# cvlab-dresden/DSAC

Measured on AMD Instinct MI355X. Metric: hypotheses scored/sec over 640x480 coord map, higher is better.
Workload: dtype f32

## Files before the change

### dsac_amd/csrc/api.hip

```cpp
#include "../../include/dsac_hip.h"
#include "kernels.h"
#include "refstream.h"

#include <hip/hip_runtime.h>
#include <cstdarg>
#include <cstdio>
#include <algorithm>
#include <cstring>
#include <cmath>
#include <deque>
#include <string>
#include <type_traits>
#include <vector>
#if defined(_GLIBCXX_RELEASE) && _GLIBCXX_RELEASE < 11
#define DSAC_RS_DEFAULT_MODE 1
#else
#define DSAC_RS_DEFAULT_MODE 0
#endif

namespace {

thread_local std::string g_last_error;

struct DevBuf {
// ... 43 lines not shown
    dk::FrameDev F{};
    DevBuf frame_xyz, frame_uv;
    std::vector<float> cams_h;
    DevBuf cams_d;
    DevBuf cam_xyz, cam_meta, rgbd_rec, rgbd_soft_part, rgbd_scratch;
    bool have_cam = false;
    GuideTable guide, rgbd_guide;
    DevBuf guide_scratch, rgbd_guide_wm;

    DevBuf rs_states, rs_scratch, rs_small, k6_scratch;
    int rs_threads = 0, rs_mode = DSAC_RS_DEFAULT_MODE;
    int pi_refstream = 0, pi_refstream_discard0 = 0, pi_refstream_attempts = 0;
    int k6_walk_exact = 0;
    int k6_waves = 0;
    int refine_soft_form = -1;
    DevBuf soft_scratch;
    DevBuf staged, staged_lo, staged_split, soft_part, bwd_staged, dRdH, grad_part, g12_part, g6;
    int g6_n = 0;
    std::deque<DevBuf> slots;
    size_t slot_next = 0;
    struct Pending { void* host; const void* dev; size_t bytes; };
    std::vector<Pending> pending;
    dk::K2Opts k2;
    int k2_last[2] = {0, 0};
    dk::K1Opts k1;
    int k1_cus = 0;
    bool device_args = false;
    int seed_stride = 1;
    int k4_variant = -1;
    hipEvent_t k2_wait = nullptr, k2_record = nullptr;

    hipStream_t aux = nullptr, aux2 = nullptr;
    DevBuf slot_staged[2], slot_soft_part[2];
    hipEvent_t slot_ready[2] = {nullptr, nullptr}, slot_free[2] = {nullptr, nullptr}, slot_reduced[2] = {nullptr, nullptr},
               slot_done[2] = {nullptr, nullptr};
    bool slot_free_recorded[2] = {false, false}, slot_reduced_recorded[2] = {false, false}, slot_done_recorded[2] = {false, false};
    bool slot_pending[2] = {false, false};
    int slot_N[2] = {0, 0};
    dk::FrameDev slot_F[2]{};
    hipEvent_t frame_ready = nullptr;

    int pi_defer_tail = 0;
    hipStream_t tail[2] = {nullptr, nullptr};
    hipEvent_t tail_go = nullptr, tail_done[2] = {nullptr, nullptr};
    bool tail_pending[2] = {false, false};
    DevBuf pi_soft[2], pi_scores[2];
// ... 159 lines not shown
    if (sums && !part) return fail(c, DSAC_ERR_INVALID, "k2_stage: the plan writes partial sums and no buffer was given");
    if (gated && c->k2_wait) HIP_TRY(c, hipStreamWaitEvent(st, c->k2_wait, 0));
    dk::K2Call call;
    if (plan.need_split) {
        HIP_TRY(c, c->staged_split.reserve(dk::pose_split_bytes(N)));
        HIP_TRY(c, dk::pose_prep_split(st, N, poses, F, c->staged_split.as<char>(), Nf));
        call.split = c->staged_split.as<char>();
    }
    if (plan.need_lo) {
        HIP_TRY(c, c->staged_lo.reserve((size_t)N * dk::POSE_STRIDE * sizeof(float)));
        HIP_TRY(c, dk::pose_prep_lo(st, N, poses, F, c->staged_lo.as<float>(), Nf));
        call.staged_lo = c->staged_lo.as<float>();
    }
    ProfScope ps(c, 0, true);
    call.poses64 = poses;
    call.diag = c->k2.diag;
    if (ps.on) { call.ev_start = ps.p.a; call.ev_stop = ps.p.b; }
    else call.ev_stop = fallback_stop;
    if (done) *done = call.ev_stop;
    HIP_TRY(c, dk::reproject(st, plan, N, staged, F, clampv, static_cast<float*>(err), tau, beta, sums ? part : nullptr, call));
    ps.commit();
    c->k2_last[0] = plan.form;
    c->k2_last[1] = plan.why;
    if (gated && c->k2_record) HIP_TRY(c, hipEventRecord(c->k2_record, st));
    return DSAC_OK;
}

struct FdStage {
    int skip = 0;
    float eps_hyp = 0.f, eps_obj = 0.f;
    dk::FdLists L{};
    dk::FdReplicas rep{};
};
int fd_stage_check(dsac_ctx* c, const char* who, float sub_sample, const float* eps_hyp, float eps_obj, FdStage* s) {
    if (eps_hyp) {
        if (!(sub_sample > 0.f) || !(*eps_hyp > 0.f) || !(eps_obj > 0.f)) return fail(c, DSAC_ERR_INVALID, "%s: sub_sample, eps_hyp, eps_obj must be > 0", who);
        s->eps_hyp = *eps_hyp;
    } else if (!(sub_sample > 0.f) || !(eps_obj > 0.f)) return fail(c, DSAC_ERR_INVALID, "%s: sub_sample and eps_obj must be > 0", who);
    s->eps_obj = eps_obj;
    s->skip = (int)(1 / sub_sample);
    if (s->skip < 1) return fail(c, DSAC_ERR_INVALID, "%s: sub_sample > 1", who);
    return DSAC_OK;
}
int fd_stage_begin(dsac_ctx* c, FdStage* s, const dk::FdLists& L, const double* init_poses, const int32_t* sets, const int32_t* maps, const int32_t* perm, int steps,
                   int max_inl, int min_inl, float thr, int32_t* obj_pixels, int32_t* n_obj, hipEvent_t planned = nullptr) {
    s->L = L;
// ... 211 lines not shown
        return fail(nullptr, DSAC_ERR_NO_DEVICE, "dsac_create: no HIP device (%s); this engine has no CPU fallback",
                    e != hipSuccess ? hipGetErrorString(e) : "device count 0");
    }
    if (device < 0 || device >= count) return fail(nullptr, DSAC_ERR_INVALID, "dsac_create: device %d out of range [0,%d)", device, count);
    HIP_TRY(nullptr, hipSetDevice(device));
    dsac_ctx* c = new (std::nothrow) dsac_ctx();
    if (!c) return fail(nullptr, DSAC_ERR_ALLOC, "dsac_create: out of host memory");
    c->device = device;
    e = hipGetDeviceProperties(&c->prop, device);
    if (e != hipSuccess) { delete c; return fail(nullptr, DSAC_ERR_HIP, "hipGetDeviceProperties: %s", hipGetErrorString(e)); }
    if (strncmp(c->prop.gcnArchName, "gfx950", 6) != 0) {
        std::string n = c->prop.gcnArchName;
        delete c;
        return fail(nullptr, DSAC_ERR_NO_DEVICE, "dsac_create: device %d is %s; this library carries gfx950 code only", device, n.c_str());
    }
    e = hipStreamCreateWithFlags(&c->stream, hipStreamNonBlocking);
    if (e != hipSuccess) { delete c; return fail(nullptr, DSAC_ERR_HIP, "hipStreamCreate: %s", hipGetErrorString(e)); }
    c->own_stream = true;
    if (const char* v = getenv("DSAC_K2_VARIANT")) c->k2.variant = atoi(v);
    if (const char* v = getenv("DSAC_TAIL_PRIO")) c->tail_prio = atoi(v) != 0;
    if (const char* v = getenv("DSAC_K2_ORDER")) c->k2.pixel_minor = atoi(v) != 0;
    if (const char* v = getenv("DSAC_K2_FLAGS")) c->k2.flags = atoi(v);
    if (const char* v = getenv("DSAC_K2_EXACT_AUTO")) c->k2.exact_auto = atoi(v) != 0;
    if (const char* v = getenv("DSAC_K1_WPB")) c->k1.wpb = atoi(v);
    if (const char* v = getenv("DSAC_K1_PRIO")) c->k1.prio = atoi(v);
    if (const char* v = getenv("DSAC_K1_HPW")) c->k1.hpw = atoi(v);
    if (const char* v = getenv("DSAC_K1_HORN")) c->k1.horn = atoi(v) != 0;
    if (const char* v = getenv("DSAC_K1_MINW")) c->k1.minw = atoi(v);
    if (const char* v = getenv("DSAC_K1_RL")) c->k1.rl = atoi(v) == 1 ? 1 : 4;
    if (const char* v = getenv("DSAC_K1_WIDE")) c->k1.wide = atoi(v);
    if (const char* v = getenv("DSAC_K1_SHARE")) { const int sv = atoi(v); c->k1.share = sv < 0 ? -sv : sv; c->k1.share_always = sv < 0; }
    if (const char* v = getenv("DSAC_K4_VARIANT")) c->k4_variant = atoi(v);
    if (const char* v = getenv("DSAC_K1_CUS")) c->k1_cus = atoi(v);
    *out = c;
    return DSAC_OK;
}

void dsac_destroy(dsac_ctx* c) {
    if (!c) return;
    (void)hipSetDevice(c->device);
    if (c->stream) (void)hipStreamSynchronize(c->stream);
    for (int k = 0; k < 2; k++)
        if (c->tail[k]) (void)hipStreamSynchronize(c->tail[k]);
    if (c->aux) (void)hipStreamSynchronize(c->aux);
    if (c->aux2) (void)hipStreamSynchronize(c->aux2);
    c->frame_xyz.release(); c->frame_uv.release(); c->cams_d.release();
// ... 739 lines not shown
    const int32_t* d_sets;
    double* d_J;
    ARG_TRY(in_arg(c, sets, (size_t)N * 4, &d_sets));
    ARG_TRY(out_arg(c, J, (size_t)N * 72, &d_J));
    HIP_TRY(c, dk::dpnp(c->stream, N, d_sets, c->F, eps, d_J, c->F.frames > 1 ? N / c->F.frames : 0));
    return end_call(c);
}

int dsac_set_option(dsac_ctx* c, const char* key, int value) {
    if (!c || !key) return fail(c, DSAC_ERR_INVALID, "dsac_set_option: NULL argument");
    const std::string k = key;
    if (k == "k2_variant") {
        if (!dk::k2_variant_known(value)) return fail(c, DSAC_ERR_INVALID, "dsac_set_option: unknown K2 kernel form %d", value);
        c->k2.variant = value;
    }
    else if (k == "k2_order") c->k2.pixel_minor = value != 0;
    else if (k == "k2_flags") c->k2.flags = value;
    else if (k == "k2_diag") c->k2.diag = value;
    else if (k == "k2_exact_auto") c->k2.exact_auto = value != 0;
    else if (k == "k2_f16_store") {
        if (value != 0 && value != 1) return fail(c, DSAC_ERR_INVALID, "dsac_set_option: k2_f16_store (both 16-bit builds, binary16 and bfloat16) is 0 (8-byte stores) or 1 (16-byte stores after a lane exchange)");
        c->k2.f16_store = value;
    }
    else if (k == "k6_walk_exact") c->k6_walk_exact = value != 0;
    else if (k == "k6_scan_tune") {
        const int g = value & 255, chunk = (value >> 8) & 0xffff;
        if ((g != 0 && g != 1 && g != 2 && g != 4) || chunk % 256 != 0 || (value >> 25) != 0) return fail(c, DSAC_ERR_INVALID, "dsac_set_option: k6_scan_tune is g | chunk << 8 | noskip << 24 with g in {0, 1, 2, 4} and chunk a multiple of 256");
        dk::refine_scan_tune(value);
    }
    else if (k == "k6_waves") {
        if (value != 0 && value != 1 && value != 2 && value != 4 && value != 8) return fail(c, DSAC_ERR_INVALID, "dsac_set_option: k6_waves is 0 (auto), 1, 2, 4 or 8");
        c->k6_waves = value;
    }
    else if (k == "refine_soft_form") {
        if (value < -1 || value > 1) return fail(c, DSAC_ERR_INVALID, "dsac_set_option: refine_soft_form is -1 (by the map size), 0 (split) or 1 (fused)");
        c->refine_soft_form = value;
    }
    else if (k == "refstream_mode") {
        if (value < -1 || value > 1) return fail(c, DSAC_ERR_INVALID, "dsac_set_option: refstream_mode is 0 (libstdc++ >= 11), 1 (libstdc++ <= 10) or -1 (this build's)");
        c->rs_mode = value < 0 ? DSAC_RS_DEFAULT_MODE : value;
    }
    else if (k == "pi_refstream") c->pi_refstream = value != 0;
    else if (k == "pi_refstream_discard0") {
        if (value < 0 || (unsigned long long)value > RS_MAX_DISCARD0) return fail(c, DSAC_ERR_INVALID, "dsac_set_option: pi_refstream_discard0 is 0 .. 2^24 outputs");
        c->pi_refstream_discard0 = value;
    }
// ... 29 lines not shown
    }
    else if (k == "k1_cus") { if (c->aux) return fail(c, DSAC_ERR_INVALID, "dsac_set_option: k1_cus must be set before the first dsac_sample_ahead"); c->k1_cus = value; }
    else return fail(c, DSAC_ERR_INVALID, "dsac_set_option: unknown key '%s'", key);
    return DSAC_OK;
}

static_assert(DSAC_K2_FORM_NONE == dk::K2_FORM_NONE && DSAC_K2_FORM_FP32_VALU == dk::K2_FORM_FP32_VALU && DSAC_K2_FORM_FP32_MFMA == dk::K2_FORM_FP32_MFMA &&
              DSAC_K2_FORM_RECLO == dk::K2_FORM_RECLO && DSAC_K2_FORM_EXACT_VEC == dk::K2_FORM_EXACT_VEC && DSAC_K2_FORM_EXACT_ANY == dk::K2_FORM_EXACT_ANY &&
              DSAC_K2_FORM_PRECISE == dk::K2_FORM_PRECISE, "enum dsac_k2_form follows the kernels' own numbering");
static_assert(DSAC_K2_WHY_AUTO_OFF == dk::K2_WHY_AUTO_OFF && DSAC_K2_WHY_FORCED == dk::K2_WHY_FORCED && DSAC_K2_WHY_FOCAL == dk::K2_WHY_FOCAL &&
              DSAC_K2_WHY_NO_POSES == dk::K2_WHY_NO_POSES, "the reason bits follow the kernels' own numbering");

int dsac_get_option(dsac_ctx* c, const char* key, int* value) {
    if (!c || !key || !value) return fail(c, DSAC_ERR_INVALID, "dsac_get_option: NULL argument");
    const std::string k = key;
    if (k == "k2_form_last") *value = c->k2_last[0];
    else if (k == "k2_form_why_last") *value = c->k2_last[1];
    else if (k == "k2_variant") *value = c->k2.variant;
    else if (k == "k2_order") *value = c->k2.pixel_minor ? 1 : 0;
    else if (k == "k2_flags") *value = c->k2.flags;
    else if (k == "k2_diag") *value = c->k2.diag;
    else if (k == "k2_exact_auto") *value = c->k2.exact_auto ? 1 : 0;
    else if (k == "k2_f16_store") *value = c->k2.f16_store;
    else if (k == "k6_walk_exact") *value = c->k6_walk_exact;
    else if (k == "k6_scan_tune") *value = dk::refine_scan_tune_get();
    else if (k == "k6_waves") *value = c->k6_waves;
    else if (k == "refine_soft_form") *value = c->refine_soft_form;
    else if (k == "refstream_mode") *value = c->rs_mode;
    else if (k == "pi_refstream") *value = c->pi_refstream;
    else if (k == "pi_refstream_discard0") *value = c->pi_refstream_discard0;
    else if (k == "pi_refstream_attempts") *value = c->pi_refstream_attempts;
    else if (k == "k1_wpb") *value = c->k1.wpb;
    else if (k == "k1_prio") *value = c->k1.prio;
    else if (k == "k1_hpw") *value = c->k1.hpw;
    else if (k == "k1_horn") *value = c->k1.horn ? 1 : 0;
    else if (k == "k1_minw") *value = c->k1.minw;
    else if (k == "k1_rl") *value = c->k1.rl;
    else if (k == "k1_wide") *value = c->k1.wide;
    else if (k == "k1_share") *value = c->k1.share_always ? -c->k1.share : c->k1.share;
    else if (k == "k4_variant") *value = c->k4_variant;
    else if (k == "device_args") *value = c->device_args ? 1 : 0;
    else if (k == "tail_prio") *value = c->tail_prio;
    else if (k == "seed_stride") *value = c->seed_stride;
    else if (k == "pi_defer_tail") *value = c->pi_defer_tail;
    else if (k == "k1_cus") *value = c->k1_cus;
    else if (k == "sampling_weights") *value = (c->have_frame && guided(c)) ? 1 : 0;
// ... 1208 lines not shown
```

### dsac_amd/csrc/k2_plan.h

```cpp
#pragma once

namespace dk {

struct K2Opts {
    bool pixel_minor = true;
    int flags = 0;
    int variant = -1;
    bool exact_auto = true;
    int diag = 0;
    int f16_store = 1;
};
enum { K2_ELEM_F32 = 0, K2_ELEM_F16 = 1, K2_ELEM_BF16 = 2 };
constexpr int K2_FLAG_STORE_ONLY = 1 << 1;
constexpr int K2_FLAG_ERR_UNFUSED = 1 << 24;
constexpr int K2_FLAG_PRECISE = 1 << 25;
constexpr int K2_FLAG_REC32 = 1 << 26;
constexpr int K2_FLAG_RECLO = 1 << 27;
constexpr int K2_FLAG_EXACT = 1 << 28;
constexpr int K2_FLAG_EXACT_ANY = 1 << 29;
constexpr int K2_FLAG_GENERAL_PATH = 1 << 30;
enum { K2_FORM_NONE = 0, K2_FORM_FP32_VALU = 1, K2_FORM_FP32_MFMA = 2, K2_FORM_RECLO = 3, K2_FORM_EXACT_VEC = 4, K2_FORM_EXACT_ANY = 5, K2_FORM_PRECISE = 6 };
enum { K2_WHY_AUTO_OFF = 1, K2_WHY_FORCED = 2, K2_WHY_FOCAL = 4, K2_WHY_NO_POSES = 8 };
constexpr int K2_NF_MULTIPLE = 128;
constexpr int K2_WG = 256;

inline bool k2_wants_exact(const K2Opts& o) {
    if (o.flags & (K2_FLAG_EXACT | K2_FLAG_EXACT_ANY)) return true;
    return o.exact_auto && o.variant < 0 && !(o.flags & (K2_FLAG_PRECISE | K2_FLAG_RECLO | K2_FLAG_STORE_ONLY | K2_FLAG_REC32));
}

enum { K2_EXONLY_OK = 0, K2_EXONLY_VARIANT = 1, K2_EXONLY_FLAGS = 2, K2_EXONLY_AUTO_OFF = 3 };
inline int k2_exact_only(int variant, int flags, bool exact_auto) {
    const int ex_bits = K2_FLAG_EXACT | K2_FLAG_EXACT_ANY;
    if (variant != -1) return K2_EXONLY_VARIANT;
    if (flags & ~(ex_bits | K2_FLAG_GENERAL_PATH)) return K2_EXONLY_FLAGS;
    if (!exact_auto && !(flags & ex_bits)) return K2_EXONLY_AUTO_OFF;
    return K2_EXONLY_OK;
}

constexpr double K2_BIG_BYTES = 1.0e9, K2_HUGE_BYTES = 4.4e9;
inline double k2_err_bytes(int N, int P) { return (double)N * (double)P * 4.0; }
constexpr int K2_SMALL_MAP_CELLS = 16384;

inline bool k2_fuse_sums(const K2Opts& o, int N, int P, bool want_err, bool want_soft) {
    return !want_soft && want_err && o.variant < 0 && !(o.flags & K2_FLAG_ERR_UNFUSED) && k2_err_bytes(N, P) > K2_BIG_BYTES;
}
// ... 81 lines not shown

struct K2PlanIn {
    K2Opts o;
    int N = 0, Nf = 0, frames = 1;
    int P = 0, W = 0;
    bool uv = false;
    bool xyz_al16 = true, uv_al16 = true, err_al16 = true;
    bool focal_ok = true;
    bool poses = true;
    bool want_err = false, want_soft = false;
    int err_elem = K2_ELEM_F32;
};
constexpr int K2_STATUS_OK = 0, K2_STATUS_INVALID = 1, K2_STATUS_NOT_SUPPORTED = 801;
struct K2Plan {
    int status = K2_STATUS_OK;
    int form = K2_FORM_NONE, why = 0;
    K2Kernel k;
    bool need_split = false, need_lo = false;
    bool fuse_sums = false;
    int kflags = 0;
    bool pixel_minor = true;
    int Nf = 0;
    int tiles = 0;
};

inline K2Plan k2_plan(const K2PlanIn& in) {
    K2Plan p;
    const K2Opts& o = in.o;
    const bool fuse = k2_fuse_sums(o, in.N, in.P, in.want_err, in.want_soft);
    const bool err = in.want_err, soft = in.want_soft || fuse;
    if (in.N <= 0 || in.P <= 0 || (!err && !soft)) return p;
    auto refuse = [](int status) { K2Plan r; r.status = status; return r; };
    if (in.Nf <= 0 || in.frames <= 1) p.Nf = ((in.N + 127) / 128) * 128;
    else if (in.Nf % K2_NF_MULTIPLE != 0) return refuse(K2_STATUS_INVALID);
    else p.Nf = in.Nf;
    p.fuse_sums = fuse;
    const int variant = o.variant;
    const bool vec = in.P % 4 == 0 && in.err_al16 && in.xyz_al16 && in.uv_al16;
    p.kflags = o.flags | ((variant >= 40 && !o.pixel_minor) ? 32 : 0);
    p.pixel_minor = o.pixel_minor;
    const bool split_ok = in.poses && k2_wants_exact(o) && in.focal_ok;
    const K2Kernel exk = k2_exact_kernel(variant), lok = k2_reclo_kernel(variant);
    const bool ex_variant = exk.family != K2_FAM_NONE;
    int why = 0;
    if (!(o.flags & (K2_FLAG_EXACT | K2_FLAG_EXACT_ANY))) {
        if (variant >= 0 || (o.flags & (K2_FLAG_PRECISE | K2_FLAG_RECLO | K2_FLAG_STORE_ONLY | K2_FLAG_REC32))) why |= K2_WHY_FORCED;
        else if (!o.exact_auto) why |= K2_WHY_AUTO_OFF;
// ... 30 lines not shown
        p.k.family = vec ? K2_FAM_EXACT_VEC : K2_FAM_EXACT_ANY;
        p.need_split = true;
        p.kflags |= 32;
    } else if (!vec) {
        p.form = K2_FORM_FP32_VALU;
        p.k.family = K2_FAM_VALU_SCALAR;
    } else {
        int id = variant;
        if (variant < 0) {
            const double bytes = k2_err_bytes(in.N, in.P);
            const bool big = bytes > K2_BIG_BYTES;
            const bool grid64 = !in.uv && (in.W & 63) == 0;
            id = soft ? (big ? ((grid64 && bytes > K2_HUGE_BYTES) ? 58 : 45) : 42) : 0;
            if (soft && big) p.kflags |= 32;
            p.pixel_minor = true;
        }
        p.k = k2_fp32_kernel(id);
        if (p.k.family == K2_FAM_NONE) return refuse(K2_STATUS_INVALID);
        if (p.k.family == K2_FAM_PS && in.N % 4 != 0 && soft) return refuse(K2_STATUS_INVALID);
        p.form = (variant < 0 ? !soft : variant <= 13) ? K2_FORM_FP32_VALU : K2_FORM_FP32_MFMA;
    }
    p.why = (p.form == K2_FORM_EXACT_VEC || p.form == K2_FORM_EXACT_ANY) ? 0 : why;
    p.tiles = k2_tiles(p.k, in.P, soft);
    return p;
}

}
```

### dsac_amd/csrc/k_forward.hip

```cpp
#include "kernels.h"
#include <hip/hip_ext.h>
#include "dmath.h"

namespace dk {

typedef float f4 __attribute__((ext_vector_type(4)));
typedef float f2 __attribute__((ext_vector_type(2)));
typedef _Float16 h4 __attribute__((ext_vector_type(4)));

DM_INLINE void pose_focal(const float4* __restrict__ cams, int h, int Nf, float& fx, float& fy) {
    if (!cams) return;
    const float4 k = cams[Nf > 0 ? h / Nf : 0];
    fx = k.x; fy = k.y;
}
DM_INLINE int split_exponent_of(float fx, float fy) {
    int e = 0;
    while (e < 31 && (float)(1u << e) < fmaxf(fx, fy)) e++;
    return e;
}
__global__ __launch_bounds__(256) void k_pose_prep(int N, const double* __restrict__ poses, float fx, float fy, float* __restrict__ staged,
                                                   const float4* __restrict__ cams, int Nf) {
    const int h = blockIdx.x * blockDim.x + threadIdx.x;
    if (h >= N) return;
    pose_focal(cams, h, Nf, fx, fy);
// ... 657 lines not shown
                                                             float* __restrict__ soft_part, int N, int P, int W, int PT, float cx, float cy,
                                                             float clampv, float kA, float kB, int kflags, int Nf, long long xyz_stride,
                                                             long long uv_stride, const float* __restrict__ staged_lo = nullptr,
                                                             const void* __restrict__ split = nullptr, const float4* __restrict__ cams = nullptr) {
    constexpr int HT = 16 * NG;
    constexpr bool EX = EXF != 0, RSQ = EXF >= 2;
    constexpr bool BF16 = EXF >= 5;
    constexpr int H16 = EXF >= 5 ? EXF - 4 : EXF >= 3 ? EXF - 2 : 0;
    static_assert(H16 == 0 || (ERR && ANY == 0 && !LO), "half error images: the vector build of the exact form, with an error image to store");
    const int b = blockIdx.x;
    int ht, pt;
    if (kflags & 32) { pt = b % PT; ht = b / PT; }
    else if (WAVES == 1) {
        const int q = b >> 5, sub = (b >> 3) & 3, PTG = (PT + 31) >> 5;
        ht = q / PTG;
        pt = ((q % PTG) * 8 + (b & 7)) * 4 + sub;
        if (pt >= PT) return;
    } else {
        const int q = b >> 3, PTG = (PT + 7) >> 3;
        ht = q / PTG;
        pt = (q % PTG) * 8 + (b & 7);
        if (pt >= PT) return;
    }
    const int h0 = ht * HT;
    const int nh = min(HT, N - h0);
    const int tid = threadIdx.x, lane = tid & 63;
    const int wave = __builtin_amdgcn_readfirstlane(tid >> 6);
    const int c = lane & 15, g = lane >> 4;
    {
        const int frame = h0 / Nf;
        xyz += (long long)frame * xyz_stride;
        if (UV) uv += (long long)frame * uv_stride;
        if (EX && cams) {
            const float4 k = cams[frame];
            cx = k.z; cy = k.w;
        }
    }
    __shared__ float s_soft[(SOFT && !PW) ? WAVES * HT : 1];

    float Bm[CHW][4];
    f2 ppix[G64 ? 1 : CHW][4];
    int sx0[G64 ? CHW : 1];
    float sby[G64 ? CHW : 1];
    int p0[CHW];
    bool valid[CHW];
    const int chunk0 = (pt * WAVES + wave) * CHW + (ANY == 2 ? (P - 1) >> 6 : 0);
#pragma unroll
    for (int ch = 0; ch < CHW; ch++) {
// ... 18 lines not shown
            oor[ch] = __any(o);
        }
    }
    h4 B16[LO ? CHW : 1][4];
    if (LO) {
#pragma unroll
        for (int ch = 0; ch < CHW; ch++)
#pragma unroll
            for (int m = 0; m < 4; m++) {
                const unsigned v = __builtin_bit_cast(unsigned, Bm[ch][m]);
                const auto r16 = __builtin_amdgcn_permlane16_swap(v, v, false, false);
                const auto r32 = __builtin_amdgcn_permlane32_swap(v, v, false, false);
                const unsigned u16 = r16[1], u32 = r32[1];
                const float s = 1.52587890625e-05f;
                const float X = Bm[ch][m] * s, Y = __builtin_bit_cast(float, u16) * s, Z = __builtin_bit_cast(float, u32) * s;
                const bool r0 = g == 0;
                B16[ch][m] = h4{(_Float16)(r0 ? X : 0.f), (_Float16)(r0 ? Y : 0.f), (_Float16)(r0 ? Z : 0.f), (_Float16)(r0 ? 0.00390625f : 0.f)};
            }
    }
    constexpr bool A_AHEAD = NG > 2;
    float ax[EX ? 1 : NG], ay[EX ? 1 : NG], az[EX ? 1 : NG];
    LoOps alo[LO ? NG : 1];
    ExOps aex[EX ? NG : 1];
    auto load_A = [&](int gi) {
        const int hyp = min(16 * gi + c, nh - 1);
        if (EX) {
            const h8* rc = reinterpret_cast<const h8*>(split) + (size_t)(h0 + hyp) * 12 + g;
            const h4* rh = reinterpret_cast<const h4*>(reinterpret_cast<const char*>(split) + (size_t)N * SPLIT_CROSS_BYTES) + (size_t)(h0 + hyp) * 12 + g;
            aex[gi].cx = rc[0]; aex[gi].cy = rc[4]; aex[gi].cz = rc[8];
            aex[gi].hx = rh[0]; aex[gi].hy = rh[4]; aex[gi].hz = rh[8];
            return;
        }
        const float* rec = staged + (size_t)(h0 + hyp) * POSE_STRIDE + g;
        ax[gi] = rec[0]; ay[gi] = rec[4]; az[gi] = rec[8];
        if (LO) {
            const f4* rl = reinterpret_cast<const f4*>(staged_lo + (size_t)(h0 + hyp) * POSE_STRIDE);
            const float S = (g == 0) ? 65536.f : 0.f, T = (g == 0) ? 256.f : 0.f;
            const f4 lx = rl[0], ly = rl[1], lz = rl[2];
            alo[gi].x = h4{(_Float16)(-lx.x * S), (_Float16)(-lx.y * S), (_Float16)(-lx.z * S), (_Float16)(-lx.w * T)};
            alo[gi].y = h4{(_Float16)(-ly.x * S), (_Float16)(-ly.y * S), (_Float16)(-ly.z * S), (_Float16)(-ly.w * T)};
            alo[gi].z = h4{(_Float16)(lz.x * S), (_Float16)(lz.y * S), (_Float16)(lz.z * S), (_Float16)(lz.w * T)};
        }
    };
#pragma unroll
    for (int gi = 0; gi < (A_AHEAD ? 1 : NG); gi++) load_A(gi);
#pragma unroll
    for (int ch = 0; ch < CHW; ch++) {
        if (UV) {
            constexpr int pc = G64 ? 0 : 1;
            if constexpr (ANY != 0) {
                if (valid[ch]) {
                    f4 u0, u1;
                    if constexpr (ANY != 2) {
                        const f4_a4* su = reinterpret_cast<const f4_a4*>(uv + (size_t)p0[ch] * 2);
                        u0 = su[0]; u1 = su[1];
                    } else {
                        const float* s1 = uv + (size_t)min(p0[ch] + 1, P - 1) * 2;
                        const float* s2 = uv + (size_t)min(p0[ch] + 2, P - 1) * 2;
                        const float* s3 = uv + (size_t)(P - 1) * 2;
// ... 9 lines not shown
                const f4* su = reinterpret_cast<const f4*>(uv + (size_t)p0[ch] * 2);
                const f4 u0 = su[0], u1 = su[1];
                ppix[ch * pc][0] = f2{u0.x - cx, u0.y - cy}; ppix[ch * pc][1] = f2{u0.z - cx, u0.w - cy};
                ppix[ch * pc][2] = f2{u1.x - cx, u1.y - cy}; ppix[ch * pc][3] = f2{u1.z - cx, u1.w - cy};
            } else {
                ppix[ch * pc][0] = ppix[ch * pc][1] = ppix[ch * pc][2] = ppix[ch * pc][3] = splat(0.f);
            }
        } else if (G64) {
            const int cpr = W >> 6;
            const int y = (chunk0 + ch) / cpr, xc0 = ((chunk0 + ch) - y * cpr) * 64;
            sx0[ch] = __builtin_amdgcn_readfirstlane(xc0);
            sby[ch] = __builtin_bit_cast(float, __builtin_amdgcn_readfirstlane(__builtin_bit_cast(int, (float)y - cy)));
        } else {
            constexpr int pc = G64 ? 0 : 1;
            int y = p0[ch] / W, x = p0[ch] - y * W;
#pragma unroll
            for (int m = 0; m < 4; m++) {
                ppix[ch * pc][m] = f2{(float)x - cx, (float)y - cy};
                if (++x == W) { x = 0; y++; }
            }
        }
    }

    if constexpr (EXF >= 2 && ANY == 0 && !LO && G64 && !UV && PW && MINW <= 3) {
        bool far = false;
#pragma unroll
        for (int ch = 0; ch < CHW; ch++) far = far || oor[ch];
        if (nh == HT && (chunk0 + CHW) * 64 <= P && !far && !(kflags & K2_FLAG_GENERAL_PATH)) {
            constexpr int GRP_STORES = ERR ? CHW * (H16 == 2 ? 2 : 4) : 0;
            __builtin_amdgcn_s_waitcnt(k2_vmcnt_imm(0));
#pragma unroll
            for (int gi = 0; gi < NG; gi++) {
                if (A_AHEAD && gi > 0) {
                    __builtin_amdgcn_s_waitcnt(k2_vmcnt_imm(GRP_STORES));
                    asm volatile("" : "+v"(aex[gi].cx), "+v"(aex[gi].cy), "+v"(aex[gi].cz), "+v"(aex[gi].hx), "+v"(aex[gi].hy), "+v"(aex[gi].hz));
                }
                if (A_AHEAD && gi + 1 < NG) {
                    asm volatile("" ::: "memory");
                    load_A(gi + 1);
                }
                const int hyp0 = 16 * gi + 4 * g;
                f2 ssum[4] = {splat(0.f), splat(0.f), splat(0.f), splat(0.f)};
#pragma unroll
                for (int ch = 0; ch < CHW; ch++) {
                    f4 ev[4];
                    f2 sloc[4];
                    f2 pb = f2{(float)(sx0[ch] + 4 * c) - cx, sby[ch]};
                    asm volatile("" : "+v"(pb));
#pragma unroll
                    for (int m = 0; m < 4; m++) ppix[0][m] = f2{pb.x + (float)m, pb.y};
                    if (__builtin_expect(__any(hp_chunk_ex<false, SOFT, RSQ>(aex[gi], B8[ch], ppix[0], clampv, kA, kB, ev, sloc)), 0)) {
                        (void)hp_chunk_ex<true, SOFT>(aex[gi], B8[ch], ppix[0], clampv, kA, kB, ev, sloc);
                    }
                    if (SOFT) {
                        const f2 vf = splat(1.0f);
#pragma unroll
                        for (int r = 0; r < 4; r++) ssum[r] = pk_fma(sloc[r], vf, ssum[r]);
                    }
                    if constexpr (H16 != 0) {
                        store_rows_h16<H16, BF16, true>(reinterpret_cast<_Float16*>(err) + (size_t)(h0 + 16 * gi) * P, ev, P, p0[ch], g, c, true, 4);
                    } else if (ERR) {
                        const __amdgpu_buffer_rsrc_t rsrc = __builtin_amdgcn_make_buffer_rsrc(err + (size_t)(h0 + 16 * gi) * P, 0, 0xffffffffu, 0x00020000);
                        const unsigned loff = ((unsigned)(4 * g) * (unsigned)P + (unsigned)p0[ch]) * 4u;
                        k2_stores_begin();
#pragma unroll
                        for (int r = 0; r < 4; r++) __builtin_amdgcn_raw_buffer_store_b128(__builtin_bit_cast(u4v, ev[r]), rsrc, loff, (unsigned)r * (unsigned)P * 4u, 2);
                        k2_stores_end();
                    }
                    if (ERR && !SOFT) {
                        const int ps = (kflags >> 16) & 15, pn = (kflags >> 20) & 15;
                        for (int i = 0; i < ps; i++) __builtin_amdgcn_s_sleep(1);
                        for (int i = 0; i < pn; i++) asm volatile("s_nop 15");
                    }
                }
                if (SOFT) {
                    const float s0 = row16_sum(ssum[0].x + ssum[0].y), s1 = row16_sum(ssum[1].x + ssum[1].y);
                    const float s2 = row16_sum(ssum[2].x + ssum[2].y), s3 = row16_sum(ssum[3].x + ssum[3].y);
                    if (c == 0) {
                        float* dst = soft_part + (size_t)(pt * WAVES + wave) * N + h0 + hyp0;
                        dst[0] = s0; dst[1] = s1; dst[2] = s2; dst[3] = s3;
                    }
                }
            }
            return;
        }
    }

#pragma unroll
    for (int gi = 0; gi < NG; gi++) {
        if (16 * gi >= nh) break;
        if (A_AHEAD && gi + 1 < NG) {
            asm volatile("" ::: "memory");
            load_A(gi + 1);
        }
        const float nax = EX ? 0.f : -ax[EX ? 0 : gi], nay = EX ? 0.f : -ay[EX ? 0 : gi];
        const int hyp0 = 16 * gi + 4 * g;
        bool grp_far = false;
        if constexpr (ANY != 0 && EX) grp_far = __any((float)aex[gi].hx[3] != 0.f || (float)aex[gi].hy[3] != 0.f || (float)aex[gi].hz[3] != 0.f);
        f2 ssum[4] = {splat(0.f), splat(0.f), splat(0.f), splat(0.f)};
#pragma unroll
        for (int ch = 0; ch < CHW; ch++) {
            f4 ev[4];
            f2 sloc[4];
            if (G64) {
                f2 pb = f2{(float)(sx0[ch] + 4 * c) - cx, sby[ch]};
                asm volatile("" : "+v"(pb));
#pragma unroll
                for (int m = 0; m < 4; m++) ppix[0][m] = f2{pb.x + (float)m, pb.y};
            }
            const f2 (&pp)[4] = ppix[G64 ? 0 : ch];
            if (EX) {
                if (__builtin_expect(oor[ch] || grp_far, 0)) {
                    const int hyp = min(16 * gi + c, nh - 1);
// ... 49 lines not shown
            }
            if (H16 == 0 && ERR && valid[ch] && fast_stores) {
                const __amdgpu_buffer_rsrc_t rsrc = __builtin_amdgcn_make_buffer_rsrc(err + (size_t)(h0 + 16 * gi) * P, 0, 0xffffffffu, 0x00020000);
                const unsigned loff = ((unsigned)(4 * g) * (unsigned)P + (unsigned)p0[ch]) * 4u;
                if (nh == HT) {
#pragma unroll
                    for (int r = 0; r < 4; r++) __builtin_amdgcn_raw_buffer_store_b128(__builtin_bit_cast(u4v, ev[r]), rsrc, loff, (unsigned)r * (unsigned)P * 4u, 2);
                } else {
#pragma unroll
                    for (int r = 0; r < 4; r++)
                        if (hyp0 + r < nh) __builtin_amdgcn_raw_buffer_store_b128(__builtin_bit_cast(u4v, ev[r]), rsrc, loff, (unsigned)r * (unsigned)P * 4u, 2);
                }
            }
            if (ERR && !SOFT) {
                const int ps = (kflags >> 16) & 15, pn = (kflags >> 20) & 15;
                for (int i = 0; i < ps; i++) __builtin_amdgcn_s_sleep(1);
                for (int i = 0; i < pn; i++) asm volatile("s_nop 15");
            }
        }
        if (SOFT) {
            const float s0 = row16_sum(ssum[0].x + ssum[0].y), s1 = row16_sum(ssum[1].x + ssum[1].y);
            const float s2 = row16_sum(ssum[2].x + ssum[2].y), s3 = row16_sum(ssum[3].x + ssum[3].y);
            if (c == 0) {
                float* dst = !PW ? s_soft + wave * HT + hyp0 : soft_part + (size_t)(pt * WAVES + wave) * N + h0 + hyp0;
                if (hyp0 + 0 < nh) dst[0] = s0;
                if (hyp0 + 1 < nh) dst[1] = s1;
                if (hyp0 + 2 < nh) dst[2] = s2;
                if (hyp0 + 3 < nh) dst[3] = s3;
            }
        }
    }
    if (SOFT && !PW) {
        __syncthreads();
        if (tid < nh) {
            float s = 0.f;
#pragma unroll
            for (int w = 0; w < WAVES; w++) s += s_soft[w * HT + tid];
            soft_part[(size_t)pt * N + h0 + tid] = s;
        }
    }
}

template <int NG>
struct K2Ops {
    float B[4];
    float A[NG][3];
};

template <int NG, int WAVES, bool ERR, bool SOFT, bool UV>
__global__ __launch_bounds__(WAVES * 64) void k_reproject_ps(const float* __restrict__ staged, const float* __restrict__ xyz,
                                                             const float* __restrict__ uv, float* __restrict__ err,
                                                             float* __restrict__ soft_part, int N, int P, int W, float cx, float cy,
// ... 135 lines not shown
    int per_cu = (kflags >> 8) & 0xff;
    if (per_cu <= 0) per_cu = 3;
    const int grid = ((cus * per_cu + 7) / 8) * 8;
    const bool ERR = err != nullptr, SOFT = soft_part != nullptr, UV = F.uv != nullptr;
#define DSAC_K2P(E, S, U)                                                                                                               \
    hipExtLaunchKernelGGL((k_reproject_ps<NG, WAVES, E, S, U>), dim3(grid), dim3(WAVES * 64), 0, st, evA, evB, 0, staged, F.xyz, F.uv, err,   \
                          soft_part, N, F.P, F.W, F.cx, F.cy, clampv, kA, kB, kflags, Nf, F.xyz_stride, F.uv_stride)
    if (ERR && SOFT) { if (UV) DSAC_K2P(true, true, true); else DSAC_K2P(true, true, false); }
    else if (ERR) { if (UV) DSAC_K2P(true, false, true); else DSAC_K2P(true, false, false); }
    else if (SOFT) { if (UV) DSAC_K2P(false, true, true); else DSAC_K2P(false, true, false); }
#undef DSAC_K2P
    return hipGetLastError();
}

template <int NG, int CHW, int MINW, int EX>
constexpr int k2_bf16_exf(bool soft, bool uv, bool g64) {
    if (EX >= 5 && NG == 4 && CHW == 1 && MINW == 3 && !uv && !g64) return soft ? 5 : 6;
    return EX;
}
template <int NG, int CHW, int WAVES, bool PW, int MINW = 1, bool LO = false, int EX = 0, int ANY = 0>
static hipError_t launch_reproject_st(hipStream_t st, int N, const float* staged, const FrameDev& F, float clampv, float* err, float kA, float kB,
                                      float* soft_part, int Nf, int kflags, hipEvent_t evA, hipEvent_t evB, const float* staged_lo = nullptr,
                                      const void* split = nullptr) {
    constexpr int HT = 16 * NG;
    const int tile = WAVES * CHW * 64;
    static_assert(PW || WAVES > 1, "one-wave workgroups write per-wave partial sums");
    const int PT = (F.P + tile - 1) / tile;
    const int NTa = (N + HT - 1) / HT;
    const int grid = (kflags & 32) ? PT * NTa : WAVES == 1 ? ((PT + 31) / 32) * 32 * NTa : ((PT + 7) / 8) * 8 * NTa;
    const bool ERR = err != nullptr, SOFT = soft_part != nullptr, UV = F.uv != nullptr;
    const bool G64 = !UV && (F.W & 63) == 0;
#define DSAC_K2S(E, S, U, G)                                                                                                               \
    hipExtLaunchKernelGGL((k_reproject_st<NG, CHW, WAVES, PW, E, S, U, G, MINW, LO, k2_bf16_exf<NG, CHW, MINW, EX>(S, U, G), ANY>), dim3(grid), dim3(WAVES * 64), 0, st, evA, evB, 0, staged, F.xyz, F.uv, err, \
                          soft_part, N, F.P, F.W, PT, F.cx, F.cy, clampv, kA, kB, kflags, Nf, F.xyz_stride, F.uv_stride, staged_lo, split, F.cams)
    if (ERR && SOFT) { if (UV) DSAC_K2S(true, true, true, false); else if (G64) DSAC_K2S(true, true, false, true); else DSAC_K2S(true, true, false, false); }
    else if (ERR) { if (UV) DSAC_K2S(true, false, true, false); else if (G64) DSAC_K2S(true, false, false, true); else DSAC_K2S(true, false, false, false); }
    else if (SOFT) {
        if constexpr (EX >= 3) return hipErrorInvalidValue;
        else { if (UV) DSAC_K2S(false, true, true, false); else if (G64) DSAC_K2S(false, true, false, true); else DSAC_K2S(false, true, false, false); }
    }
#undef DSAC_K2S
    return hipGetLastError();
}

template <int NG, int CHW, int MINW>
static hipError_t launch_reproject_any(hipStream_t st, int N, const float* staged, const FrameDev& F, float clampv, float* err, float kA, float kB, float* soft_part,
                                       int Nf, int kflags, hipEvent_t evA, hipEvent_t evB, const void* split) {
    const bool tail = (F.P & 3) != 0;
    const int rows = (F.P + CHW * 64 - 1) / (CHW * 64);
    hipError_t e = launch_reproject_st<NG, CHW, 1, true, MINW, false, 2, 1>(st, N, staged, F, clampv, err, kA, kB, soft_part, Nf, kflags, evA, tail ? nullptr : evB, nullptr, split);
    if (e != hipSuccess || !tail) return e;
// ... 212 lines not shown
    const int NTa = (N + HT - 1) / HT;
    const int grid = ((PT + 7) / 8) * 8 * NTa;
    const int NT = pixel_minor ? -NTa : NTa;
    const bool ERR = err != nullptr, SOFT = soft_part != nullptr, UV = F.uv != nullptr;
#define DSAC_K2(E, S, U)                                                                                                              \
    hipExtLaunchKernelGGL((k_reproject<PX, HT, E, S, U, SPOSE>), dim3(grid), dim3(K2_THREADS), 0, st, evA, evB, 0, staged, F.xyz, F.uv, err, soft_part, \
                          N, F.P, F.W, PT, NT, F.cx, F.cy, clampv, kA, kB, kflags, Nf, F.xyz_stride, F.uv_stride)
    if (ERR && SOFT) { if (UV) DSAC_K2(true, true, true); else DSAC_K2(true, true, false); }
    else if (ERR) { if (UV) DSAC_K2(true, false, true); else DSAC_K2(true, false, false); }
    else if (SOFT) { if (UV) DSAC_K2(false, true, true); else DSAC_K2(false, true, false); }
#undef DSAC_K2
    return hipGetLastError();
}

static_assert(K2_WG == K2_THREADS, "k2_plan.h counts partial-sum rows with the workgroup size of the kernels");
static_assert(K2_STATUS_OK == (int)hipSuccess && K2_STATUS_INVALID == (int)hipErrorInvalidValue && K2_STATUS_NOT_SUPPORTED == (int)hipErrorNotSupported,
              "k2_plan.h spells the HIP status values out");
hipError_t reproject(hipStream_t st, const K2Plan& plan, int N, const float* staged, const FrameDev& F, float clampv, float* err, float tau, float beta,
                     float* soft_part, const K2Call& call) {
    if (plan.status != K2_STATUS_OK) return (hipError_t)plan.status;
    const K2Kernel& k = plan.k;
    const float LOG2E = 1.4426950408889634f;
    const float kA = beta * LOG2E, kB = -beta * tau * LOG2E;
    const int Nf = plan.Nf, kf = plan.kflags;
    const bool pm = plan.pixel_minor;
    hipEvent_t evA = call.ev_start, evB = call.ev_stop;
#define DSAC_VA(PX_, HT_, SP_) launch_reproject<PX_, HT_, SP_>(st, N, staged, F, clampv, err, kA, kB, soft_part, Nf, pm, kf, evA, evB)
#define DSAC_HP(HT_, CH_) launch_reproject_hp<HT_, CH_>(st, N, staged, F, clampv, err, kA, kB, soft_part, Nf, pm, kf, evA, evB)
#define DSAC_ST(NG_, CH_, WV_, PW_, MW_) launch_reproject_st<NG_, CH_, WV_, PW_, MW_>(st, N, staged, F, clampv, err, kA, kB, soft_part, Nf, kf, evA, evB)
#define DSAC_PS(NG_) launch_reproject_ps<NG_, 4>(st, N, staged, F, clampv, err, kA, kB, soft_part, Nf, kf, evA, evB)
#define DSAC_LO(NG_, CH_, MW_) launch_reproject_st<NG_, CH_, 1, true, MW_, true>(st, N, staged, F, clampv, err, kA, kB, soft_part, Nf, kf, evA, evB, call.staged_lo)
#define DSAC_EX(NG_, CH_, MW_, F_) launch_reproject_st<NG_, CH_, 1, true, MW_, false, F_>(st, N, staged, F, clampv, err, kA, kB, soft_part, Nf, kf, evA, evB, nullptr, call.split)
#define DSAC_EXA(NG_, CH_, MW_) launch_reproject_any<NG_, CH_, MW_>(st, N, staged, F, clampv, err, kA, kB, soft_part, Nf, kf, evA, evB, call.split)
    switch (k.family) {
        case K2_FAM_NONE: return hipSuccess;
        case K2_FAM_VALU_SCALAR: return DSAC_VA(1, 32, false);
        case K2_FAM_VALU: case K2_FAM_HP: case K2_FAM_ST: case K2_FAM_PS:
            switch (k.id) {
#define K2_VA_(ID, PX, HT, SP) case ID: return DSAC_VA(PX, HT, SP);
#define K2_HP_(ID, HT, CH) case ID: return DSAC_HP(HT, CH);
#define K2_ST_(ID, NG, CH, WV, PW, MW) case ID: return DSAC_ST(NG, CH, WV, PW, MW);
#define K2_PS_(ID, NG) case ID: return DSAC_PS(NG);
                K2_FP32_IDS(K2_VA_, K2_HP_, K2_ST_, K2_PS_)
#undef K2_VA_
#undef K2_HP_
#undef K2_ST_
#undef K2_PS_
// ... 155 lines not shown
```

Measured before the change: 3.969 million.

## Let each K2 workgroup walk several hypothesis tiles over the same pixel chunk

Adds a hypothesis walk to the exact-vector reprojection kernel. Each workgroup now processes 1, 2 or 4 consecutive hypothesis tiles and reuses its pixel-side operands, prefetching the next tile's first group of pose operands while it finishes the current one. The grid shrinks by the same factor. This is meant to cut per-workgroup setup and repeated pixel loads. The walk factor is chosen automatically only for large error outputs with enough workgroups left to fill the GPU, and can be forced through an environment variable or option; it costs parallelism and adds control-flow complexity.

```diff
diff --git a/dsac_amd/csrc/api.hip b/dsac_amd/csrc/api.hip
--- a/dsac_amd/csrc/api.hip
+++ b/dsac_amd/csrc/api.hip
@@ -89,6 +89,7 @@
     struct Pending { void* host; const void* dev; size_t bytes; };
     std::vector<Pending> pending;
     dk::K2Opts k2;
+    int k2_walk_last = 0;
     int k2_last[2] = {0, 0};
     dk::K1Opts k1;
     int k1_cus = 0;
@@ -294,6 +295,7 @@
     ps.commit();
     c->k2_last[0] = plan.form;
     c->k2_last[1] = plan.why;
+    c->k2_walk_last = plan.hyp_walk;
     if (gated && c->k2_record) HIP_TRY(c, hipEventRecord(c->k2_record, st));
     return DSAC_OK;
 }
@@ -551,6 +553,7 @@
     if (const char* v = getenv("DSAC_K2_ORDER")) c->k2.pixel_minor = atoi(v) != 0;
     if (const char* v = getenv("DSAC_K2_FLAGS")) c->k2.flags = atoi(v);
     if (const char* v = getenv("DSAC_K2_EXACT_AUTO")) c->k2.exact_auto = atoi(v) != 0;
+    if (const char* v = getenv("DSAC_K2_HYP_WALK")) { const int w = atoi(v); if (w == 1 || w == 2 || w == 4) c->k2.hyp_walk = w; }
     if (const char* v = getenv("DSAC_K1_WPB")) c->k1.wpb = atoi(v);
     if (const char* v = getenv("DSAC_K1_PRIO")) c->k1.prio = atoi(v);
     if (const char* v = getenv("DSAC_K1_HPW")) c->k1.hpw = atoi(v);
@@ -1336,6 +1339,10 @@
         if (value != 0 && value != 1) return fail(c, DSAC_ERR_INVALID, "dsac_set_option: k2_f16_store (both 16-bit builds, binary16 and bfloat16) is 0 (8-byte stores) or 1 (16-byte stores after a lane exchange)");
         c->k2.f16_store = value;
     }
+    else if (k == "k2_hyp_walk") {
+        if (value != 0 && value != 1 && value != 2 && value != 4) return fail(c, DSAC_ERR_INVALID, "dsac_set_option: k2_hyp_walk is 0 (auto), 1, 2 or 4 hypothesis tiles per workgroup");
+        c->k2.hyp_walk = value;
+    }
     else if (k == "k6_walk_exact") c->k6_walk_exact = value != 0;
     else if (k == "k6_scan_tune") {
         const int g = value & 255, chunk = (value >> 8) & 0xffff;
@@ -1411,6 +1418,8 @@
     else if (k == "k2_diag") *value = c->k2.diag;
     else if (k == "k2_exact_auto") *value = c->k2.exact_auto ? 1 : 0;
     else if (k == "k2_f16_store") *value = c->k2.f16_store;
+    else if (k == "k2_hyp_walk") *value = c->k2.hyp_walk;
+    else if (k == "k2_hyp_walk_last") *value = c->k2_walk_last;
     else if (k == "k6_walk_exact") *value = c->k6_walk_exact;
     else if (k == "k6_scan_tune") *value = dk::refine_scan_tune_get();
     else if (k == "k6_waves") *value = c->k6_waves;
diff --git a/dsac_amd/csrc/k2_plan.h b/dsac_amd/csrc/k2_plan.h
--- a/dsac_amd/csrc/k2_plan.h
+++ b/dsac_amd/csrc/k2_plan.h
@@ -9,6 +9,7 @@
     bool exact_auto = true;
     int diag = 0;
     int f16_store = 1;
+    int hyp_walk = 0;
 };
 enum { K2_ELEM_F32 = 0, K2_ELEM_F16 = 1, K2_ELEM_BF16 = 2 };
 constexpr int K2_FLAG_STORE_ONLY = 1 << 1;
@@ -22,6 +23,7 @@
 enum { K2_FORM_NONE = 0, K2_FORM_FP32_VALU = 1, K2_FORM_FP32_MFMA = 2, K2_FORM_RECLO = 3, K2_FORM_EXACT_VEC = 4, K2_FORM_EXACT_ANY = 5, K2_FORM_PRECISE = 6 };
 enum { K2_WHY_AUTO_OFF = 1, K2_WHY_FORCED = 2, K2_WHY_FOCAL = 4, K2_WHY_NO_POSES = 8 };
 constexpr int K2_NF_MULTIPLE = 128;
+constexpr int K2_KFLAG_WALK_SHIFT = 6;
 constexpr int K2_WG = 256;
 
 inline bool k2_wants_exact(const K2Opts& o) {
@@ -149,7 +151,32 @@
     bool pixel_minor = true;
     int Nf = 0;
     int tiles = 0;
-};
+    int hyp_walk = 1;
+};
+
+constexpr int K2_WALK_AUTO = 4;
+constexpr int K2_WAVE_SLOTS = 256 * 4 * 2;
+constexpr int K2_WALK_MIN_GENERATIONS = 8;
+inline bool k2_has_walk(const K2PlanIn& in, const K2Kernel& k) {
+    return k.family == K2_FAM_EXACT_VEC && k.exf >= 2 && k.pw && k.wv == 1 && k.minw <= 3 && !in.uv && (in.W & 63) == 0;
+}
+inline bool k2_walk_legal(const K2PlanIn& in, const K2Kernel& k, int walk) {
+    const int hyps = 16 * k.ng * walk;
+    return in.N % hyps == 0 && (in.frames <= 1 || in.Nf <= 0 || in.Nf % hyps == 0);
+}
+inline int k2_walks(int N, int ng, int walk) { return k2_ceil_div(k2_ceil_div(N, 16 * ng), walk); }
+inline int k2_hyp_walk(const K2PlanIn& in, const K2Kernel& k) {
+    if (!k2_has_walk(in, k)) return 1;
+    int walk = in.o.hyp_walk;
+    if (walk <= 0) {
+        walk = K2_WALK_AUTO;
+        if (!(k.ch == 4 && k.minw == 2 && k2_err_bytes(in.N, in.P) > K2_BIG_BYTES)) walk = 1;
+        const long long wgs = (long long)k2_ceil_div(in.N, 16 * k.ng) * k2_ceil_div(in.P, 64 * k.ch);
+        while (walk > 1 && wgs / walk < (long long)K2_WALK_MIN_GENERATIONS * K2_WAVE_SLOTS) walk >>= 1;
+    }
+    while (walk > 1 && !k2_walk_legal(in, k, walk)) walk >>= 1;
+    return walk;
+}
 
 inline K2Plan k2_plan(const K2PlanIn& in) {
     K2Plan p;
@@ -226,6 +253,7 @@
     }
     p.why = (p.form == K2_FORM_EXACT_VEC || p.form == K2_FORM_EXACT_ANY) ? 0 : why;
     p.tiles = k2_tiles(p.k, in.P, soft);
+    p.hyp_walk = k2_hyp_walk(in, p.k);
     return p;
 }
 
diff --git a/dsac_amd/csrc/k_forward.hip b/dsac_amd/csrc/k_forward.hip
--- a/dsac_amd/csrc/k_forward.hip
+++ b/dsac_amd/csrc/k_forward.hip
@@ -703,8 +703,10 @@
         pt = (q % PTG) * 8 + (b & 7);
         if (pt >= PT) return;
     }
-    const int h0 = ht * HT;
-    const int nh = min(HT, N - h0);
+    constexpr bool FULL_TILE = EXF >= 2 && ANY == 0 && !LO && G64 && !UV && PW && MINW <= 3;
+    const int HB = FULL_TILE ? 1 << ((kflags >> K2_KFLAG_WALK_SHIFT) & 3) : 1;
+    int h0 = ht * HT * HB;
+    int nh = min(HT, N - h0);
     const int tid = threadIdx.x, lane = tid & 63;
     const int wave = __builtin_amdgcn_readfirstlane(tid >> 6);
     const int c = lane & 15, g = lane >> 4;
@@ -769,19 +771,20 @@
     float ax[EX ? 1 : NG], ay[EX ? 1 : NG], az[EX ? 1 : NG];
     LoOps alo[LO ? NG : 1];
     ExOps aex[EX ? NG : 1];
+    int lh = h0, lc = c;
     auto load_A = [&](int gi) {
-        const int hyp = min(16 * gi + c, nh - 1);
+        const int hyp = min(16 * gi + lc, nh - 1);
         if (EX) {
-            const h8* rc = reinterpret_cast<const h8*>(split) + (size_t)(h0 + hyp) * 12 + g;
-            const h4* rh = reinterpret_cast<const h4*>(reinterpret_cast<const char*>(split) + (size_t)N * SPLIT_CROSS_BYTES) + (size_t)(h0 + hyp) * 12 + g;
+            const h8* rc = reinterpret_cast<const h8*>(split) + (size_t)(lh + hyp) * 12 + g;
+            const h4* rh = reinterpret_cast<const h4*>(reinterpret_cast<const char*>(split) + (size_t)N * SPLIT_CROSS_BYTES) + (size_t)(lh + hyp) * 12 + g;
             aex[gi].cx = rc[0]; aex[gi].cy = rc[4]; aex[gi].cz = rc[8];
             aex[gi].hx = rh[0]; aex[gi].hy = rh[4]; aex[gi].hz = rh[8];
             return;
         }
-        const float* rec = staged + (size_t)(h0 + hyp) * POSE_STRIDE + g;
+        const float* rec = staged + (size_t)(lh + hyp) * POSE_STRIDE + g;
         ax[gi] = rec[0]; ay[gi] = rec[4]; az[gi] = rec[8];
         if (LO) {
-            const f4* rl = reinterpret_cast<const f4*>(staged_lo + (size_t)(h0 + hyp) * POSE_STRIDE);
+            const f4* rl = reinterpret_cast<const f4*>(staged_lo + (size_t)(lh + hyp) * POSE_STRIDE);
             const float S = (g == 0) ? 65536.f : 0.f, T = (g == 0) ? 256.f : 0.f;
             const f4 lx = rl[0], ly = rl[1], lz = rl[2];
             alo[gi].x = h4{(_Float16)(-lx.x * S), (_Float16)(-lx.y * S), (_Float16)(-lx.z * S), (_Float16)(-lx.w * T)};
@@ -837,73 +840,94 @@
         }
     }
 
-    if constexpr (EXF >= 2 && ANY == 0 && !LO && G64 && !UV && PW && MINW <= 3) {
+    if constexpr (FULL_TILE) {
         bool far = false;
 #pragma unroll
         for (int ch = 0; ch < CHW; ch++) far = far || oor[ch];
         if (nh == HT && (chunk0 + CHW) * 64 <= P && !far && !(kflags & K2_FLAG_GENERAL_PATH)) {
             constexpr int GRP_STORES = ERR ? CHW * (H16 == 2 ? 2 : 4) : 0;
             __builtin_amdgcn_s_waitcnt(k2_vmcnt_imm(0));
-#pragma unroll
-            for (int gi = 0; gi < NG; gi++) {
-                if (A_AHEAD && gi > 0) {
-                    __builtin_amdgcn_s_waitcnt(k2_vmcnt_imm(GRP_STORES));
-                    asm volatile("" : "+v"(aex[gi].cx), "+v"(aex[gi].cy), "+v"(aex[gi].cz), "+v"(aex[gi].hx), "+v"(aex[gi].hy), "+v"(aex[gi].hz));
-                }
-                if (A_AHEAD && gi + 1 < NG) {
-                    asm volatile("" ::: "memory");
-                    load_A(gi + 1);
-                }
-                const int hyp0 = 16 * gi + 4 * g;
-                f2 ssum[4] = {splat(0.f), splat(0.f), splat(0.f), splat(0.f)};
-#pragma unroll
-                for (int ch = 0; ch < CHW; ch++) {
-                    f4 ev[4];
-                    f2 sloc[4];
-                    f2 pb = f2{(float)(sx0[ch] + 4 * c) - cx, sby[ch]};
-                    asm volatile("" : "+v"(pb));
-#pragma unroll
-                    for (int m = 0; m < 4; m++) ppix[0][m] = f2{pb.x + (float)m, pb.y};
-                    if (__builtin_expect(__any(hp_chunk_ex<false, SOFT, RSQ>(aex[gi], B8[ch], ppix[0], clampv, kA, kB, ev, sloc)), 0)) {
-                        (void)hp_chunk_ex<true, SOFT>(aex[gi], B8[ch], ppix[0], clampv, kA, kB, ev, sloc);
+            static_assert(A_AHEAD, "the walk fetches the next tile's first group from the last group of this one");
+#pragma unroll 1
+            for (int k = 0;; k++) {
+                __builtin_amdgcn_s_waitcnt(k2_vmcnt_imm(GRP_STORES));
+                asm volatile("" : "+v"(aex[0].cx), "+v"(aex[0].cy), "+v"(aex[0].cz), "+v"(aex[0].hx), "+v"(aex[0].hy), "+v"(aex[0].hz));
+#pragma unroll
+                for (int gi = 0; gi < NG; gi++) {
+                    if (A_AHEAD && gi > 0) {
+                        __builtin_amdgcn_s_waitcnt(k2_vmcnt_imm(GRP_STORES));
+                        asm volatile("" : "+v"(aex[gi].cx), "+v"(aex[gi].cy), "+v"(aex[gi].cz), "+v"(aex[gi].hx), "+v"(aex[gi].hy), "+v"(aex[gi].hz));
+                    }
+                    lh = h0; lc = c;
+                    asm volatile("" : "+s"(lh), "+v"(lc));
+                    const int hk = lh;
+                    if (A_AHEAD && gi + 1 < NG) {
+                        asm volatile("" ::: "memory");
+                        load_A(gi + 1);
+                    } else if (k + 1 < HB) {
+                        asm volatile("" ::: "memory");
+                        lh += HT;
+                        load_A(0);
+                    }
+                    const int hyp0 = 16 * gi + 4 * g;
+                    f2 ssum[4] = {splat(0.f), splat(0.f), splat(0.f), splat(0.f)};
+#pragma unroll
+                    for (int ch = 0; ch < CHW; ch++) {
+                        f4 ev[4];
+                        f2 sloc[4];
+                        f2 pb = f2{(float)(sx0[ch] + 4 * c) - cx, sby[ch]};
+                        asm volatile("" : "+v"(pb));
+#pragma unroll
+                        for (int m = 0; m < 4; m++) ppix[0][m] = f2{pb.x + (float)m, pb.y};
+                        if (__builtin_expect(__any(hp_chunk_ex<false, SOFT, RSQ>(aex[gi], B8[ch], ppix[0], clampv, kA, kB, ev, sloc)), 0)) {
+                            (void)hp_chunk_ex<true, SOFT>(aex[gi], B8[ch], ppix[0], clampv, kA, kB, ev, sloc);
+                        }
+                        if (SOFT) {
+                            const f2 vf = splat(1.0f);
+#pragma unroll
+                            for (int r = 0; r < 4; r++) ssum[r] = pk_fma(sloc[r], vf, ssum[r]);
+                        }
+                        if constexpr (H16 != 0) {
+                            store_rows_h16<H16, BF16, true>(reinterpret_cast<_Float16*>(err) + (size_t)(h0 + 16 * gi) * P, ev, P, p0[ch], g, c, true, 4);
+                        } else if (ERR) {
+                            const __amdgpu_buffer_rsrc_t rsrc = __builtin_amdgcn_make_buffer_rsrc(err + (size_t)(h0 + 16 * gi) * P, 0, 0xffffffffu, 0x00020000);
+                            const unsigned loff = ((unsigned)(4 * g) * (unsigned)P + (unsigned)p0[ch]) * 4u;
+                            k2_stores_begin();
+#pragma unroll
+                            for (int r = 0; r < 4; r++) __builtin_amdgcn_raw_buffer_store_b128(__builtin_bit_cast(u4v, ev[r]), rsrc, loff, (unsigned)r * (unsigned)P * 4u, 2);
+                            k2_stores_end();
+                        }
+                        if (ERR && !SOFT) {
+                            const int ps = (kflags >> 16) & 15, pn = (kflags >> 20) & 15;
+                            for (int i = 0; i < ps; i++) __builtin_amdgcn_s_sleep(1);
+                            for (int i = 0; i < pn; i++) asm volatile("s_nop 15");
+                        }
                     }
                     if (SOFT) {
-                        const f2 vf = splat(1.0f);
-#pragma unroll
-                        for (int r = 0; r < 4; r++) ssum[r] = pk_fma(sloc[r], vf, ssum[r]);
-                    }
-                    if constexpr (H16 != 0) {
-                        store_rows_h16<H16, BF16, true>(reinterpret_cast<_Float16*>(err) + (size_t)(h0 + 16 * gi) * P, ev, P, p0[ch], g, c, true, 4);
-                    } else if (ERR) {
-                        const __amdgpu_buffer_rsrc_t rsrc = __builtin_amdgcn_make_buffer_rsrc(err + (size_t)(h0 + 16 * gi) * P, 0, 0xffffffffu, 0x00020000);
-                        const unsigned loff = ((unsigned)(4 * g) * (unsigned)P + (unsigned)p0[ch]) * 4u;
-                        k2_stores_begin();
-#pragma unroll
-                        for (int r = 0; r < 4; r++) __builtin_amdgcn_raw_buffer_store_b128(__builtin_bit_cast(u4v, ev[r]), rsrc, loff, (unsigned)r * (unsigned)P * 4u, 2);
-                        k2_stores_end();
-                    }
-                    if (ERR && !SOFT) {
-                        const int ps = (kflags >> 16) & 15, pn = (kflags >> 20) & 15;
-                        for (int i = 0; i < ps; i++) __builtin_amdgcn_s_sleep(1);
-                        for (int i = 0; i < pn; i++) asm volatile("s_nop 15");
+                        const float s0 = row16_sum(ssum[0].x + ssum[0].y), s1 = row16_sum(ssum[1].x + ssum[1].y);
+                        const float s2 = row16_sum(ssum[2].x + ssum[2].y), s3 = row16_sum(ssum[3].x + ssum[3].y);
+                        if (c == 0) {
+                            float* dst = soft_part + (size_t)(pt * WAVES + wave) * N + hk + hyp0;
+                            dst[0] = s0; dst[1] = s1; dst[2] = s2; dst[3] = s3;
+                        }
                     }
                 }
-                if (SOFT) {
-                    const float s0 = row16_sum(ssum[0].x + ssum[0].y), s1 = row16_sum(ssum[1].x + ssum[1].y);
-                    const float s2 = row16_sum(ssum[2].x + ssum[2].y), s3 = row16_sum(ssum[3].x + ssum[3].y);
-                    if (c == 0) {
-                        float* dst = soft_part + (size_t)(pt * WAVES + wave) * N + h0 + hyp0;
-                        dst[0] = s0; dst[1] = s1; dst[2] = s2; dst[3] = s3;
-                    }
-                }
+                if (k + 1 == HB) break;
+                h0 += HT;
             }
             return;
         }
     }
 
+    [[maybe_unused]] int walked = 1;
+[[maybe_unused]] next_tile:;
 #pragma unroll
     for (int gi = 0; gi < NG; gi++) {
         if (16 * gi >= nh) break;
+        if constexpr (FULL_TILE) {
+            lh = h0; lc = c;
+            asm volatile("" : "+s"(lh), "+v"(lc));
+        }
         if (A_AHEAD && gi + 1 < NG) {
             asm volatile("" ::: "memory");
             load_A(gi + 1);
@@ -999,12 +1023,23 @@
             const float s0 = row16_sum(ssum[0].x + ssum[0].y), s1 = row16_sum(ssum[1].x + ssum[1].y);
             const float s2 = row16_sum(ssum[2].x + ssum[2].y), s3 = row16_sum(ssum[3].x + ssum[3].y);
             if (c == 0) {
-                float* dst = !PW ? s_soft + wave * HT + hyp0 : soft_part + (size_t)(pt * WAVES + wave) * N + h0 + hyp0;
+                float* dst = !PW ? s_soft + wave * HT + hyp0 : soft_part + (size_t)(pt * WAVES + wave) * N + (FULL_TILE ? lh : h0) + hyp0;
                 if (hyp0 + 0 < nh) dst[0] = s0;
                 if (hyp0 + 1 < nh) dst[1] = s1;
                 if (hyp0 + 2 < nh) dst[2] = s2;
                 if (hyp0 + 3 < nh) dst[3] = s3;
             }
+        }
+    }
+    if constexpr (FULL_TILE) {
+        static_assert(A_AHEAD, "a further tile starts with the operands of its first group alone");
+        if (walked < HB) {
+            walked++;
+            h0 += HT;
+            nh = min(HT, N - h0);
+            lh = h0;
+            load_A(0);
+            goto next_tile;
         }
     }
     if (SOFT && !PW) {
@@ -1186,11 +1221,10 @@
 static hipError_t launch_reproject_st(hipStream_t st, int N, const float* staged, const FrameDev& F, float clampv, float* err, float kA, float kB,
                                       float* soft_part, int Nf, int kflags, hipEvent_t evA, hipEvent_t evB, const float* staged_lo = nullptr,
                                       const void* split = nullptr) {
-    constexpr int HT = 16 * NG;
     const int tile = WAVES * CHW * 64;
     static_assert(PW || WAVES > 1, "one-wave workgroups write per-wave partial sums");
     const int PT = (F.P + tile - 1) / tile;
-    const int NTa = (N + HT - 1) / HT;
+    const int NTa = k2_walks(N, NG, 1 << ((kflags >> K2_KFLAG_WALK_SHIFT) & 3));
     const int grid = (kflags & 32) ? PT * NTa : WAVES == 1 ? ((PT + 31) / 32) * 32 * NTa : ((PT + 7) / 8) * 8 * NTa;
     const bool ERR = err != nullptr, SOFT = soft_part != nullptr, UV = F.uv != nullptr;
     const bool G64 = !UV && (F.W & 63) == 0;
@@ -1449,7 +1483,7 @@
     const K2Kernel& k = plan.k;
     const float LOG2E = 1.4426950408889634f;
     const float kA = beta * LOG2E, kB = -beta * tau * LOG2E;
-    const int Nf = plan.Nf, kf = plan.kflags;
+    const int Nf = plan.Nf, kf = (plan.kflags & ~(3 << K2_KFLAG_WALK_SHIFT)) | ((plan.hyp_walk == 4 ? 2 : plan.hyp_walk == 2 ? 1 : 0) << K2_KFLAG_WALK_SHIFT);
     const bool pm = plan.pixel_minor;
     hipEvent_t evA = call.ev_start, evB = call.ev_stop;
 #define DSAC_VA(PX_, HT_, SP_) launch_reproject<PX_, HT_, SP_>(st, N, staged, F, clampv, err, kA, kB, soft_part, Nf, pm, kf, evA, evB)
```

Result: faster. 4.089 million (median of 6 runs) (+3.0%).
